# FutureSDR/FutureSDR

Hardware: NVIDIA H100
Metric: Msamples/s (higher is better)
Workload: dtype f32

## Files before the change

### futuresdr_b200/csrc/fir.cuh

```cuda
#pragma once
#include "common.cuh"

struct b2s_fir {
    b2s_ctx *ctx = nullptr;
    b2s_kind kind = B2S_C32_F32;
    size_t ntaps = 0, decim = 1;
    std::vector<float> taps_host;
    b2s_algo algo_req = B2S_ALGO_AUTO, algo = B2S_ALGO_DIRECT;

    Buf<float> d_ptaps;
    int Upad = 0;

    int tc_kblocks = 0;
    bool tc_ready = false;
    int tc_flags = 0;

    Buf<float2> d_fftH;

    Buf<double> d_taps64;
};

int32_t fir_direct_prepare(b2s_fir *f);
int32_t fir_direct_launch(b2s_fir *f, const void *d_in, size_t n_in, void *d_out, size_t n_out,
                          cudaStream_t stream);
std::vector<float> slide_table(const float *taps, size_t tf, size_t L, size_t M, size_t T, size_t lead);
bool    resamp_slide_supported(size_t L, size_t M, size_t T, size_t item_bytes);
int32_t resamp_slide_launch(b2s_ctx *ctx, b2s_kind kind, const float *d_gtab, size_t L, size_t M, size_t T,
                            const void *d_in, size_t n_in, void *d_out, size_t n_out, cudaStream_t stream);
struct FirHist {
    const void *d_hist = nullptr;
    size_t n_hist = 0;
    unsigned *publish_flag = nullptr;
    unsigned publish_value = 0;
    const unsigned *wait_flag = nullptr;
    unsigned wait_value = 0;
    unsigned *done_flag = nullptr;
    unsigned done_value = 0;
};
bool    fir_tc_supported(const b2s_fir *f);
int32_t fir_tc_launch_hist(b2s_fir *f, const FirHist *h, const void *d_in, size_t n_in, void *d_out, size_t n_out,
                           cudaStream_t stream);
int32_t fir_tc_prepare(b2s_fir *f);
int32_t fir_tc_launch(b2s_fir *f, const void *d_in, size_t n_in, void *d_out, size_t n_out,
                      cudaStream_t stream);
int32_t fir_f64_prepare(b2s_fir *f, const double *taps);
int32_t fir_f64_launch(b2s_fir *f, const void *d_in, size_t n_in, void *d_out, size_t n_out, cudaStream_t stream);
bool    fir_fft_supported(const b2s_fir *f);
int32_t fir_fft_prepare(b2s_fir *f);
int32_t fir_fft_launch(b2s_fir *f, const void *d_in, size_t n_in, void *d_out, size_t n_out,
                       cudaStream_t stream);
```

### futuresdr_b200/csrc/fir_tc.cu

```cuda
#include <cuda_bf16.h>

#include <algorithm>
#include <climits>
#include <cstdlib>
#include <type_traits>

#include "fir.cuh"

namespace {

constexpr int kStages = 2;
#ifndef B2S_RAW_SLOTS
#define B2S_RAW_SLOTS 6
#endif
constexpr int kRawSlots = B2S_RAW_SLOTS;
constexpr int kRawSlotBytes = 8192;
constexpr int kNumProducerThreads = 256;
constexpr int kNumMathThreads = 256;
constexpr int kNumLoaderThreads = 128;
constexpr int kThreadsTC = kNumMathThreads + kNumProducerThreads + kNumLoaderThreads;
constexpr int kProdWarps = kNumProducerThreads / 32;
constexpr int kMathWarps = kNumMathThreads / 32;
constexpr int kProdWarp0 = kMathWarps;
constexpr int kTmaWarp = kProdWarp0 + kProdWarps;
constexpr int kRegsAtLaunch = 65536 / kThreadsTC / 8 * 8;
constexpr int kMathRegs = 176, kProdRegs = 48, kLoaderRegs = 24;
static_assert(kNumMathThreads * kMathRegs + kNumProducerThreads * kProdRegs + kNumLoaderThreads * kLoaderRegs <=
              kThreadsTC * kRegsAtLaunch, "setmaxnreg budget exceeds the CTA's register allocation");
constexpr int kAtomsOut = 16;
constexpr int kMaxDK = 3;
constexpr int kMaxKSteps = (63 + 128 * kMaxDK - 128) / 16 + 1;
constexpr int kSplitBytesMax = (kAtomsOut + kMaxDK - 1) * 1024 * 2;
constexpr int kStageBytes = 2 * kSplitBytesMax;
constexpr int kACores = kMaxDK * 16 + 15;
constexpr int kABytes = kACores * 128;
constexpr int kSmemTC = kStages * kStageBytes + kRawSlots * kRawSlotBytes + 2 * kABytes + 1024  + 256 ;
static_assert(kSmemTC <= 227 * 1024, "tensor FIR shared memory exceeds the 227 KiB per-CTA limit");

__device__ __forceinline__ uint32_t smem_u32(const void *p) { return (uint32_t)__cvta_generic_to_shared(p); }

__device__ __forceinline__ void mbar_init(uint32_t bar, uint32_t count) {
    asm volatile("mbarrier.init.shared::cta.b64 [%0], %1;" ::"r"(bar), "r"(count));
}
__device__ __forceinline__ void mbar_arrive(uint32_t bar) {
    asm volatile("mbarrier.arrive.shared::cta.b64 _, [%0];" ::"r"(bar) : "memory");
}
__device__ __forceinline__ bool mbar_try_wait(uint32_t bar, uint32_t parity) {
    uint32_t ok;
    asm volatile(
        "{\n\t.reg .pred p;\n\t"
        "mbarrier.try_wait.parity.shared::cta.b64 p, [%1], %2;\n\t"
        "selp.b32 %0, 1, 0, p;\n\t}"
        : "=r"(ok) : "r"(bar), "r"(parity) : "memory");
    return ok != 0;
}
__device__ __forceinline__ void mbar_wait(uint32_t bar, uint32_t parity) {
    while (!mbar_try_wait(bar, parity)) {}
}
__device__ __forceinline__ bool elect_one() {
    uint32_t pred;
    asm volatile("{\n\t.reg .pred p;\n\telect.sync _|p, 0xffffffff;\n\tselp.b32 %0, 1, 0, p;\n\t}" : "=r"(pred));
    return pred != 0;
}
__device__ __forceinline__ void fence_barrier_init() { asm volatile("fence.mbarrier_init.release.cluster;" ::: "memory"); }
__device__ __forceinline__ void fence_proxy_async() { asm volatile("fence.proxy.async.shared::cta;" ::: "memory"); }

__device__ __forceinline__ void wgmma_fence() { asm volatile("wgmma.fence.sync.aligned;" ::: "memory"); }
__device__ __forceinline__ void wgmma_commit() { asm volatile("wgmma.commit_group.sync.aligned;" ::: "memory"); }
__device__ __forceinline__ void wgmma_wait_all() { asm volatile("wgmma.wait_group.sync.aligned 0;" ::: "memory"); }
__device__ __forceinline__ void st_global_if(float2 *p, float a, float b, bool pred) {
    asm volatile("{\n\t.reg .pred q;\n\tsetp.ne.b32 q, %3, 0;\n\t@q st.global.v2.f32 [%0], {%1, %2};\n\t}"
                 ::"l"(p), "f"(a), "f"(b), "r"((int)pred) : "memory");
}
__device__ __forceinline__ void st_global_if(float *p, float a, bool pred) {
    asm volatile("{\n\t.reg .pred q;\n\tsetp.ne.b32 q, %2, 0;\n\t@q st.global.f32 [%0], %1;\n\t}"
                 ::"l"(p), "f"(a), "r"((int)pred) : "memory");
}
template <int R> __device__ __forceinline__ void setmaxnreg_inc() { asm volatile("setmaxnreg.inc.sync.aligned.u32 %0;" ::"n"(R)); }
template <int R> __device__ __forceinline__ void setmaxnreg_dec() { asm volatile("setmaxnreg.dec.sync.aligned.u32 %0;" ::"n"(R)); }
__device__ __forceinline__ void wgmma_m64n128(float (&d)[64], uint64_t a_desc, uint64_t b_desc, uint32_t accumulate) {
    asm volatile(
        "{\n\t.reg .pred p;\n\t"
        "setp.ne.b32 p, %66, 0;\n\t"
        "wgmma.mma_async.sync.aligned.m64n128k16.f32.bf16.bf16 "
        "{%0, %1, %2, %3, %4, %5, %6, %7, %8, %9, %10, %11, %12, %13, %14, %15, %16, %17, %18, %19, %20, %21, %22, "
        "%23, %24, %25, %26, %27, %28, %29, %30, %31, %32, %33, %34, %35, %36, %37, %38, %39, %40, %41, %42, %43, "
        "%44, %45, %46, %47, %48, %49, %50, %51, %52, %53, %54, %55, %56, %57, %58, %59, %60, %61, %62, %63}, "
        "%64, %65, p, 1, 1, 0, 0;\n\t}"
        : "+f"(d[0]), "+f"(d[1]), "+f"(d[2]), "+f"(d[3]), "+f"(d[4]), "+f"(d[5]), "+f"(d[6]), "+f"(d[7]),
          "+f"(d[8]), "+f"(d[9]), "+f"(d[10]), "+f"(d[11]), "+f"(d[12]), "+f"(d[13]), "+f"(d[14]), "+f"(d[15]),
          "+f"(d[16]), "+f"(d[17]), "+f"(d[18]), "+f"(d[19]), "+f"(d[20]), "+f"(d[21]), "+f"(d[22]), "+f"(d[23]),
          "+f"(d[24]), "+f"(d[25]), "+f"(d[26]), "+f"(d[27]), "+f"(d[28]), "+f"(d[29]), "+f"(d[30]), "+f"(d[31]),
          "+f"(d[32]), "+f"(d[33]), "+f"(d[34]), "+f"(d[35]), "+f"(d[36]), "+f"(d[37]), "+f"(d[38]), "+f"(d[39]),
          "+f"(d[40]), "+f"(d[41]), "+f"(d[42]), "+f"(d[43]), "+f"(d[44]), "+f"(d[45]), "+f"(d[46]), "+f"(d[47]),
          "+f"(d[48]), "+f"(d[49]), "+f"(d[50]), "+f"(d[51]), "+f"(d[52]), "+f"(d[53]), "+f"(d[54]), "+f"(d[55]),
          "+f"(d[56]), "+f"(d[57]), "+f"(d[58]), "+f"(d[59]), "+f"(d[60]), "+f"(d[61]), "+f"(d[62]), "+f"(d[63])
        : "l"(a_desc), "l"(b_desc), "r"(accumulate)
        : "memory");
}
__device__ __forceinline__ void wgmma_m64n128_rs(float (&d)[64], const uint32_t (&a)[4], uint64_t b_desc,
                                                 uint32_t accumulate) {
    asm volatile(
        "{\n\t.reg .pred p;\n\t"
        "setp.ne.b32 p, %69, 0;\n\t"
        "wgmma.mma_async.sync.aligned.m64n128k16.f32.bf16.bf16 "
        "{%0, %1, %2, %3, %4, %5, %6, %7, %8, %9, %10, %11, %12, %13, %14, %15, %16, %17, %18, %19, %20, %21, %22, "
        "%23, %24, %25, %26, %27, %28, %29, %30, %31, %32, %33, %34, %35, %36, %37, %38, %39, %40, %41, %42, %43, "
        "%44, %45, %46, %47, %48, %49, %50, %51, %52, %53, %54, %55, %56, %57, %58, %59, %60, %61, %62, %63}, "
        "{%64, %65, %66, %67}, %68, p, 1, 1, 0;\n\t}"
        : "+f"(d[0]), "+f"(d[1]), "+f"(d[2]), "+f"(d[3]), "+f"(d[4]), "+f"(d[5]), "+f"(d[6]), "+f"(d[7]),
          "+f"(d[8]), "+f"(d[9]), "+f"(d[10]), "+f"(d[11]), "+f"(d[12]), "+f"(d[13]), "+f"(d[14]), "+f"(d[15]),
          "+f"(d[16]), "+f"(d[17]), "+f"(d[18]), "+f"(d[19]), "+f"(d[20]), "+f"(d[21]), "+f"(d[22]), "+f"(d[23]),
          "+f"(d[24]), "+f"(d[25]), "+f"(d[26]), "+f"(d[27]), "+f"(d[28]), "+f"(d[29]), "+f"(d[30]), "+f"(d[31]),
          "+f"(d[32]), "+f"(d[33]), "+f"(d[34]), "+f"(d[35]), "+f"(d[36]), "+f"(d[37]), "+f"(d[38]), "+f"(d[39]),
          "+f"(d[40]), "+f"(d[41]), "+f"(d[42]), "+f"(d[43]), "+f"(d[44]), "+f"(d[45]), "+f"(d[46]), "+f"(d[47]),
          "+f"(d[48]), "+f"(d[49]), "+f"(d[50]), "+f"(d[51]), "+f"(d[52]), "+f"(d[53]), "+f"(d[54]), "+f"(d[55]),
          "+f"(d[56]), "+f"(d[57]), "+f"(d[58]), "+f"(d[59]), "+f"(d[60]), "+f"(d[61]), "+f"(d[62]), "+f"(d[63])
        : "r"(a[0]), "r"(a[1]), "r"(a[2]), "r"(a[3]), "l"(b_desc), "r"(accumulate)
        : "memory");
}
__device__ __forceinline__ uint32_t ld_shared_b32(uint32_t addr) {
    uint32_t v;
    asm volatile("ld.shared.b32 %0, [%1];" : "=r"(v) : "r"(addr));
    return v;
}

__device__ __forceinline__ uint32_t cvt_bf16x2(float a, float b) {
    uint32_t r;
    asm("cvt.rn.bf16x2.f32 %0, %1, %2;" : "=r"(r) : "f"(b), "f"(a));
    return r;
}
__device__ __forceinline__ void split2(float a, float b, uint32_t &hi, uint32_t &lo) {
    hi = cvt_bf16x2(a, b);
    const float ah = __uint_as_float(hi << 16), bh = __uint_as_float(hi & 0xffff0000u);
    lo = cvt_bf16x2(a - ah, b - bh);
}

__device__ __forceinline__ uint64_t make_desc(uint32_t smem_addr, uint32_t lbo, uint32_t sbo, uint32_t layout) {
    return (uint64_t)((smem_addr & 0x3FFFF) >> 4) | ((uint64_t)(lbo >> 4) << 16) | ((uint64_t)(sbo >> 4) << 32) |
           ((uint64_t)layout << 62);
}
__device__ __forceinline__ uint64_t make_b_desc(uint32_t smem_addr) { return make_desc(smem_addr, 16, 1024, 1); }
__device__ __forceinline__ uint64_t make_a_desc(uint32_t smem_addr) { return make_desc(smem_addr, 128, 128, 0); }

struct TcParams {
    const float *in;
    float *out;
    const float *g;
    long long n_in;
    long long n_out;
    int ntaps;
    int DK;
    int num_tiles;
    int flags;
    int decim;
    const float *hist;
    int hist_items;
    int lead;
    const unsigned *wait_flag;
    unsigned wait_value;
    unsigned *done_flag;
    unsigned done_value;
    unsigned *pub_flag;
    unsigned pub_value;
    unsigned *status;
};

template <bool COMPLEX>
__global__ void __launch_bounds__(kThreadsTC, 1) fir_tc_kernel(const TcParams prm) {
    extern __shared__ unsigned char smem_raw[];
    const uint32_t raw = smem_u32(smem_raw);
    const uint32_t base = (raw + 1023u) & ~1023u;
    unsigned char *gen_base = smem_raw + (base - raw);
    const uint32_t raw_base = base + kStages * kStageBytes;
    unsigned char *raw_gen = gen_base + kStages * kStageBytes;
    const uint32_t a_base = raw_base + kRawSlots * kRawSlotBytes;
    __nv_bfloat16 *a_gen = reinterpret_cast<__nv_bfloat16 *>(raw_gen + kRawSlots * kRawSlotBytes);
    const uint32_t bar_base = a_base + 2 * kABytes;
    auto full_bar = [&](int s) { return bar_base + 8u * s; };
    auto empty_bar = [&](int s) { return bar_base + 8u * (kStages + s); };
    auto rfull_bar = [&](int r) { return bar_base + 8u * (2 * kStages + r); };
    auto rempty_bar = [&](int r) { return bar_base + 8u * (2 * kStages + kRawSlots + r); };

    const int warp = threadIdx.x >> 5, lane = threadIdx.x & 31;
    if (prm.pub_flag && blockIdx.x == 0 && threadIdx.x == 0) {
        __threadfence_system();
        asm volatile("st.release.sys.global.u32 [%0], %1;" ::"l"(prm.pub_flag), "r"(prm.pub_value) : "memory");
    }
    const int DK = prm.DK, K = 128 * DK;
    const int atoms = kAtomsOut + DK - 1;
    const int chunk_bytes = atoms * 1024;
    const int split_bytes = 2 * chunk_bytes;
    constexpr int NSEQ = COMPLEX ? 4 : 8;
    constexpr int TILE_BLOCKS = kAtomsOut * NSEQ;
    constexpr long long TILE_ITEMS = (long long)TILE_BLOCKS * 128;

    if (warp == kTmaWarp && lane == 0) {
        for (int s = 0; s < kStages; s++) { mbar_init(full_bar(s), kProdWarps); mbar_init(empty_bar(s), kMathWarps); }
        for (int r = 0; r < kRawSlots; r++) { mbar_init(rfull_bar(r), 1); mbar_init(rempty_bar(r), kProdWarps); }
        fence_barrier_init();
    }
    const int a_elems = (K / 8 + 15) * 64;
    for (int i = threadIdx.x; i < a_elems; i += kThreadsTC) {
        const int s = i >> 6, r = (i >> 3) & 7, e = i & 7;
        const int t = 8 * s + r + e - 127 - prm.lead;
        const float gv = (t >= 0 && t < prm.ntaps) ? __ldg(prm.g + t) : 0.0f;
        const __nv_bfloat16 hi = __float2bfloat16_rn(gv);
        a_gen[i] = hi;
        a_gen[kABytes / 2 + i] = __float2bfloat16_rn(gv - __bfloat162float(hi));
    }
    fence_proxy_async();
    __syncthreads();

    constexpr int F4_PER_BLOCK = COMPLEX ? 64 : 32;
    constexpr int BLOCKS_PER_SLOT = 512 / F4_PER_BLOCK;
    constexpr int SLOTS_PER_TILE = (TILE_BLOCKS + kMaxDK - 1 + BLOCKS_PER_SLOT - 1) / BLOCKS_PER_SLOT;
    constexpr int ITEM_BYTES = COMPLEX ? 8 : 4;
    const int in_blocks = TILE_BLOCKS + DK - 1;

    if (warp >= kTmaWarp) {
        setmaxnreg_dec<kLoaderRegs>();
        if (warp != kTmaWarp) return;
        if (elect_one()) {
            int rs = 0;
            uint32_t rphase = 0;
            for (int tile = blockIdx.x; tile < prm.num_tiles; tile += gridDim.x) {
                const long long item0 = (long long)tile * TILE_ITEMS;
#pragma unroll 1
                for (int s = 0; s < SLOTS_PER_TILE; s++) {
                    const int blk_first = s * BLOCKS_PER_SLOT;
                    if (blk_first >= in_blocks) break;
                    const int nblk = min(BLOCKS_PER_SLOT, in_blocks - blk_first);
                    const long long it0 = item0 + (long long)blk_first * 128;
                    long long items = (long long)nblk * 128;
                    if (it0 + items > prm.n_in) items = prm.n_in - it0;
                    long long bytes = items > 0 ? ((items * ITEM_BYTES) & ~15ll) : 0;
                    mbar_wait(rempty_bar(rs), rphase ^ 1);
                    if (tile == 0 && s == 0 && prm.hist_items > 0) {
                        if (prm.wait_flag) {
                            unsigned long long t0, t1;
                            asm volatile("mov.u64 %0, %%globaltimer;" : "=l"(t0));
                            for (;;) {
                                unsigned v;
                                asm volatile("ld.acquire.sys.global.u32 %0, [%1];" : "=r"(v) : "l"(prm.wait_flag) : "memory");
                                if ((int)(v - prm.wait_value) >= 0) break;
                                asm volatile("mov.u64 %0, %%globaltimer;" : "=l"(t1));
                                if (t1 - t0 > 4000000000ull) { atomicOr(prm.status, 1u); break; }
                                __nanosleep(64);
                            }
                            asm volatile("fence.proxy.async;" ::: "memory");
                        }
                        const uint32_t hb = (uint32_t)prm.hist_items * ITEM_BYTES;
                        const uint32_t rest = bytes > (long long)hb ? (uint32_t)bytes - hb : 0u;
                        asm volatile("mbarrier.arrive.expect_tx.shared::cta.b64 _, [%0], %1;" ::"r"(rfull_bar(rs)), "r"(hb + rest) : "memory");
                        asm volatile("cp.async.bulk.shared::cluster.global.mbarrier::complete_tx::bytes [%0], [%1], %2, [%3];"
                                     ::"r"(raw_base + rs * kRawSlotBytes), "l"(prm.hist), "r"(hb), "r"(rfull_bar(rs)) : "memory");
                        if (rest)
                            asm volatile("cp.async.bulk.shared::cluster.global.mbarrier::complete_tx::bytes [%0], [%1], %2, [%3];"
                                         ::"r"(raw_base + rs * kRawSlotBytes + hb), "l"(prm.in + (COMPLEX ? 2 : 1) * (long long)prm.hist_items),
                                           "r"(rest), "r"(rfull_bar(rs)) : "memory");
                    } else if (bytes > 0) {
                        asm volatile("mbarrier.arrive.expect_tx.shared::cta.b64 _, [%0], %1;" ::"r"(rfull_bar(rs)), "r"((uint32_t)bytes) : "memory");
                        asm volatile("cp.async.bulk.shared::cluster.global.mbarrier::complete_tx::bytes [%0], [%1], %2, [%3];"
                                     ::"r"(raw_base + rs * kRawSlotBytes), "l"(prm.in + (COMPLEX ? 2 : 1) * it0),
                                       "r"((uint32_t)bytes), "r"(rfull_bar(rs)) : "memory");
                    } else {
                        mbar_arrive(rfull_bar(rs));
                    }
                    if (++rs == kRawSlots) { rs = 0; rphase ^= 1; }
                }
            }
        }
        __syncwarp();
    } else if (warp >= kProdWarp0) {
        setmaxnreg_dec<kProdRegs>();
        const int tid = threadIdx.x - 32 * kProdWarp0;
        const int fo = tid % F4_PER_BLOCK, rowsel = tid / F4_PER_BLOCK;
        const int kc = COMPLEX ? (fo >> 5) : (fo >> 4);
        const int c16 = COMPLEX ? ((fo & 31) >> 2) : ((fo & 15) >> 1);
        const int wofs = COMPLEX ? (fo & 3) * 4 : (fo & 1) * 8;
        const uint32_t t_off = (uint32_t)(kc * chunk_bytes + wofs + rowsel * 1024);
        uint32_t xj[8];
#pragma unroll
        for (int j = 0; j < 8; j++) xj[j] = (uint32_t)(j * 128 + ((c16 ^ j) << 4));
        const bool alias_thread = rowsel < DK - 1;
        const uint32_t sb = (uint32_t)split_bytes;

        auto convert_tile = [&](auto interior_c, unsigned char *stage_ptr, long long item0, int &rs, uint32_t &rphase) {
            constexpr bool INTERIOR = decltype(interior_c)::value;
            unsigned char *tp = stage_ptr + t_off;
#pragma unroll
            for (int s = 0; s < SLOTS_PER_TILE; s++) {
                if (s * BLOCKS_PER_SLOT >= in_blocks) break;
                mbar_wait(rfull_bar(rs), rphase);
                const float4 *raw = reinterpret_cast<const float4 *>(raw_gen + rs * kRawSlotBytes);
                float4 v[2];
                v[0] = raw[tid];
                v[1] = raw[tid + 256];
                const int rs_cur = rs;
                if (++rs == kRawSlots) { rs = 0; rphase ^= 1; }
                if constexpr (!INTERIOR) {
                    if (s == 0 && item0 == 0 && tid == 0 && prm.done_flag)
                        asm volatile("st.release.sys.global.u32 [%0], %1;" ::"l"(prm.done_flag), "r"(prm.done_value) : "memory");
                }
#pragma unroll
                for (int i = 0; i < 2; i++) {
                    constexpr int ROWS = COMPLEX ? 4 : 8;
                    const int g_ct = COMPLEX ? (8 * (s & 1) + 4 * i) : (8 * i);
                    const int seq = COMPLEX ? (s >> 1) : s;
                    const bool alias_ct = COMPLEX ? ((s & 1) == 0 && i == 0 && s >= 2) : (i == 0 && s >= 1);
                    if (s == SLOTS_PER_TILE - 1) {
                        if (s * BLOCKS_PER_SLOT + rowsel + ROWS * i >= in_blocks) continue;
                    }
                    if (prm.flags & 8) continue;
                    if constexpr (!INTERIOR) {
                        const int bl = s * BLOCKS_PER_SLOT + rowsel + ROWS * i;
                        const long long it = item0 + (long long)bl * 128 + (long long)fo * (COMPLEX ? 2 : 4);
                        const long long gf = it * (COMPLEX ? 2 : 1);
                        const long long total_f = prm.n_in * (COMPLEX ? 2 : 1), copied_f = total_f & ~3ll;
                        float *e = reinterpret_cast<float *>(&v[i]);
                        const long long lead_f = (long long)prm.lead * (COMPLEX ? 2 : 1);
#pragma unroll
                        for (int c = 0; c < 4; c++) {
                            if (gf + c >= total_f || gf + c < lead_f) e[c] = 0.0f;
                            else if (gf + c >= copied_f) e[c] = prm.in[gf + c];
                        }
                    }
                    if constexpr (COMPLEX) {
                        uint32_t rh, rl, ih, il;
                        split2(v[i].x, v[i].z, rh, rl);
                        split2(v[i].y, v[i].w, ih, il);
                        if (seq < NSEQ) {
                            unsigned char *q = tp + g_ct * 1024;
                            *reinterpret_cast<uint32_t *>(q + xj[2 * (seq & 3)]) = rh;
                            *reinterpret_cast<uint32_t *>(q + xj[2 * (seq & 3)] + sb) = rl;
                            *reinterpret_cast<uint32_t *>(q + xj[2 * (seq & 3) + 1]) = ih;
                            *reinterpret_cast<uint32_t *>(q + xj[2 * (seq & 3) + 1] + sb) = il;
                        }
                        if (alias_ct && alias_thread) {
                            unsigned char *q = tp + (g_ct + kAtomsOut) * 1024;
                            *reinterpret_cast<uint32_t *>(q + xj[2 * ((seq - 1) & 3)]) = rh;
                            *reinterpret_cast<uint32_t *>(q + xj[2 * ((seq - 1) & 3)] + sb) = rl;
                            *reinterpret_cast<uint32_t *>(q + xj[2 * ((seq - 1) & 3) + 1]) = ih;
                            *reinterpret_cast<uint32_t *>(q + xj[2 * ((seq - 1) & 3) + 1] + sb) = il;
                        }
                    } else {
                        uint32_t h0, l0, h1, l1;
                        split2(v[i].x, v[i].y, h0, l0);
                        split2(v[i].z, v[i].w, h1, l1);
                        if (seq < NSEQ) {
                            unsigned char *q = tp + g_ct * 1024 + xj[seq & 7];
                            *reinterpret_cast<uint2 *>(q) = make_uint2(h0, h1);
                            *reinterpret_cast<uint2 *>(q + sb) = make_uint2(l0, l1);
                        }
                        if (alias_ct && alias_thread) {
                            unsigned char *q = tp + (g_ct + kAtomsOut) * 1024 + xj[(seq - 1) & 7];
                            *reinterpret_cast<uint2 *>(q) = make_uint2(h0, h1);
                            *reinterpret_cast<uint2 *>(q + sb) = make_uint2(l0, l1);
                        }
                    }
                }
                __syncwarp();
                if (lane == 0) mbar_arrive(rempty_bar(rs_cur));
            }
        };

        int stage = 0, rs = 0;
        uint32_t phase = 0, rphase = 0;
        for (int tile = blockIdx.x; tile < prm.num_tiles; tile += gridDim.x) {
            const long long item0 = (long long)tile * TILE_ITEMS;
            const bool interior = item0 + (long long)in_blocks * 128 <= prm.n_in &&
                                  !(tile == 0 && (prm.lead | prm.hist_items) != 0);
            mbar_wait(empty_bar(stage), phase ^ 1);
            unsigned char *stage_ptr = gen_base + stage * kStageBytes;
            if (interior) convert_tile(std::true_type{}, stage_ptr, item0, rs, rphase);
            else convert_tile(std::false_type{}, stage_ptr, item0, rs, rphase);
            fence_proxy_async();
            __syncwarp();
            if (lane == 0) mbar_arrive(full_bar(stage));
            if (++stage == kStages) { stage = 0; phase ^= 1; }
        }
    } else {
        setmaxnreg_inc<kMathRegs>();
        const int wg = __shfl_sync(0xffffffffu, warp >> 2, 0);
        const int wl = warp & 3, q4 = lane & 3;
        const int D = prm.decim, per_blk = 128 / D;
        const uint32_t a_hi = a_base + 1024u * wg, a_lo = a_hi + kABytes;
        const int p0 = 64 * (1 - wg);
        const int j0 = p0 / 16;
        const int nsteps = (prm.flags & 4) ? 0 : min((p0 + 63 + prm.lead + prm.ntaps - 1) / 16, 8 * DK - 1) - j0 + 1;

        uint32_t ghi[kMaxKSteps][4];
        {
            const uint32_t f0 = a_hi + 256u * (uint32_t)(wl + j0) + 16u * (uint32_t)(lane >> 2) + 4u * (uint32_t)q4;
#pragma unroll
            for (int i = 0; i < kMaxKSteps; i++) {
                const uint32_t f = f0 + 256u * i;
                const bool used = i < nsteps;
                ghi[i][0] = used ? ld_shared_b32(f) : 0u;
                ghi[i][1] = used ? ld_shared_b32(f + 128u) : 0u;
                ghi[i][2] = used ? ld_shared_b32(f + 128u) : 0u;
                ghi[i][3] = used ? ld_shared_b32(f + 256u) : 0u;
            }
        }

        const uint64_t a_lo_desc = make_a_desc(a_lo + 256u * j0);

        int stage = 0;
        uint32_t phase = 0;
        auto mma_tile = [&](float (&acc)[64]) {
            mbar_wait(full_bar(stage), phase);
            wgmma_fence();
            const uint64_t b_desc = make_b_desc(base + stage * kStageBytes);
#pragma unroll
            for (int i = 0; i < kMaxKSteps; i++) {
                if (i >= nsteps) break;
                const int m = (j0 >> 2) + (i >> 2);
                const uint64_t bh = b_desc + (uint32_t)(((m & 1) * chunk_bytes + (m >> 1) * 1024 + (i & 3) * 32) >> 4);
                wgmma_m64n128_rs(acc, ghi[i], bh, i != 0);
                wgmma_m64n128_rs(acc, ghi[i], bh + (uint32_t)(split_bytes >> 4), 1u);
                wgmma_m64n128(acc, a_lo_desc + 16u * i, bh, 1u);
            }
            wgmma_commit();
        };
        auto release_stage = [&]() {
            wgmma_wait_all();
            __syncwarp();
            if (lane == 0) mbar_arrive(empty_bar(stage));
            if (++stage == kStages) { stage = 0; phase ^= 1; }
        };
        const int log2D = __ffs(D) - 1;
        auto store_tile = [&](const float (&acc)[64], int tile) {
            if (prm.flags & 2) return;
#pragma unroll
            for (int h = 0; h < 2; h++) {
                const int p = 127 - (64 * wg + 16 * wl + (lane >> 2) + 8 * h);
                const int keep = (p & (D - 1)) == D - 1;
                const long long kb = ((long long)tile * TILE_BLOCKS + kAtomsOut * q4 * (COMPLEX ? 1 : 2)) * per_blk +
                                     (p >> log2D);
                const int room = (int)max(min(prm.n_out - kb, (long long)INT_MAX), 0ll) & -keep;
                const int ncols = (int)(((unsigned)room + (unsigned)per_blk - 1u) >> (7 - log2D));
                if constexpr (COMPLEX) {
#pragma unroll
                    for (int gam = 0; gam < 16; gam++)
                        st_global_if(reinterpret_cast<float2 *>(prm.out) + kb + gam * per_blk, acc[4 * gam + 2 * h],
                                     acc[4 * gam + 2 * h + 1], gam < ncols);
                } else {
#pragma unroll
                    for (int n = 0; n < 2 * kAtomsOut; n++)
                        st_global_if(prm.out + (kb + n * per_blk), acc[4 * (n % kAtomsOut) + 2 * h + n / kAtomsOut],
                                     n < ncols);
                }
            }
        };

        float acc[64];
#pragma unroll
        for (int i = 0; i < 64; i++) acc[i] = 0.0f;
        for (int tile = blockIdx.x; tile < prm.num_tiles; tile += gridDim.x) {
            mma_tile(acc);
            release_stage();
            store_tile(acc, tile);
        }
    }
}

}

bool fir_tc_supported(const b2s_fir *f) {
    if (f->decim == 0 || f->decim > 128 || 128 % f->decim != 0) return false;
    if (f->kind != B2S_C32_F32 && f->kind != B2S_F32_F32) return false;
    return f->ntaps >= 16 && f->ntaps <= 128 * kMaxDK - 127;
}

int32_t fir_tc_prepare(b2s_fir *f) {
    b2s_ctx *ctx = f->ctx;
    if (f->tc_ready) return B2S_OK;
    if (!fir_tc_supported(f)) return b2s_fail(ctx, B2S_EUNSUPPORTED, "tensor FIR: unsupported plan");
    f->tc_kblocks = (int)ceil_div(f->ntaps + 127, 128);
    B2S_CUDA(ctx, cudaFuncSetAttribute(fir_tc_kernel<true>, cudaFuncAttributeMaxDynamicSharedMemorySize, kSmemTC));
    B2S_CUDA(ctx, cudaFuncSetAttribute(fir_tc_kernel<false>, cudaFuncAttributeMaxDynamicSharedMemorySize, kSmemTC));
    for (const void *k : {(const void *)fir_tc_kernel<true>, (const void *)fir_tc_kernel<false>}) {
        cudaFuncAttributes attr;
        B2S_CUDA(ctx, cudaFuncGetAttributes(&attr, k));
        if (attr.numRegs != kRegsAtLaunch)
            return b2s_fail(ctx, B2S_EUNSUPPORTED, "tensor FIR: kernel built with %d registers per thread, its setmaxnreg "
                            "budget assumes %d", attr.numRegs, kRegsAtLaunch);
    }
    if (const char *e = getenv("B2S_TC_FLAGS")) f->tc_flags = atoi(e);
    f->tc_ready = true;
    return B2S_OK;
}

int32_t fir_tc_launch_hist(b2s_fir *f, const FirHist *h, const void *d_in, size_t n_in, void *d_out, size_t n_out,
                           cudaStream_t stream) {
    b2s_ctx *ctx = f->ctx;
    if (n_out == 0) return B2S_OK;
    if (!f->tc_ready) return b2s_fail(ctx, B2S_ESTATE, "tensor FIR not prepared");
    const bool cplx = f->kind == B2S_C32_F32;
    const size_t item = cplx ? 8 : 4, q = 16 / item;
    const uintptr_t a_in = reinterpret_cast<uintptr_t>(d_in), a_out = reinterpret_cast<uintptr_t>(d_out);
    if ((a_in % item) || (a_out % item)) return B2S_EAGAIN;
    const size_t n_hist = h ? h->n_hist : 0;
    size_t lead;
    if (n_hist) {
        const uintptr_t a_h = reinterpret_cast<uintptr_t>(h->d_hist);
        if ((a_h % item) || (a_in & 15)) return B2S_EAGAIN;
        lead = (a_h / item) % q;
        if ((lead + n_hist) % q) return B2S_EAGAIN;
        if (lead + n_hist > 1024 || n_in * item < 16) return B2S_EAGAIN;
    } else {
        lead = (a_in / item) % q;
    }
    const int DK = (int)ceil_div(f->ntaps + lead + 127, 128);
    if (DK > kMaxDK) return B2S_EAGAIN;
    TcParams prm;
    prm.lead = (int)lead;
    prm.hist_items = n_hist ? (int)(lead + n_hist) : 0;
    prm.hist = n_hist ? (const float *)h->d_hist - lead * (item / 4) : nullptr;
    prm.in = (const float *)d_in - (lead + n_hist) * (item / 4);
    prm.wait_flag = (h && n_hist) ? h->wait_flag : nullptr;
    prm.wait_value = h ? h->wait_value : 0;
    prm.done_flag = (h && n_hist) ? h->done_flag : nullptr;
    prm.done_value = h ? h->done_value : 0;
    prm.pub_flag = h ? h->publish_flag : nullptr;
    prm.pub_value = h ? h->publish_value : 0;
    prm.status = ctx->d_status;
    prm.out = (float *)d_out;
    prm.g = f->d_ptaps.get() + (size_t)f->decim * f->Upad;
    prm.n_in = (long long)(lead + n_hist + n_in);
    prm.n_out = (long long)n_out;
    prm.decim = (int)f->decim;
    prm.ntaps = (int)f->ntaps;
    prm.DK = DK;
    const long long tile_items = cplx ? 64 * 128 : 128 * 128;
    prm.num_tiles = (int)ceil_div(n_out * f->decim, (size_t)tile_items);
    prm.flags = f->tc_flags;
    const int grid = std::min(prm.num_tiles, ctx->sm_count);
    if (prm.wait_flag) ctx->flag_ops++;
    if (cplx) fir_tc_kernel<true><<<grid, kThreadsTC, kSmemTC, stream>>>(prm);
    else fir_tc_kernel<false><<<grid, kThreadsTC, kSmemTC, stream>>>(prm);
    B2S_CHECK_LAUNCH(ctx);
    return B2S_OK;
}

int32_t fir_tc_launch(b2s_fir *f, const void *d_in, size_t n_in, void *d_out, size_t n_out,
                      cudaStream_t stream) {
    const int32_t rc = fir_tc_launch_hist(f, nullptr, d_in, n_in, d_out, n_out, stream);
    if (rc == B2S_EAGAIN) return fir_direct_launch(f, d_in, n_in, d_out, n_out, stream);
    return rc;
}
```

Before: 172,000.

## Schedule tensor FIR tiles dynamically via a global atomic counter

```diff
diff --git a/futuresdr_b200/csrc/fir.cuh b/futuresdr_b200/csrc/fir.cuh
--- a/futuresdr_b200/csrc/fir.cuh
+++ b/futuresdr_b200/csrc/fir.cuh
@@ -14,6 +14,7 @@
     int tc_kblocks = 0;
     bool tc_ready = false;
     int tc_flags = 0;
+    Buf<unsigned> d_tc_sched;
 
     Buf<float2> d_fftH;
 
diff --git a/futuresdr_b200/csrc/fir_tc.cu b/futuresdr_b200/csrc/fir_tc.cu
--- a/futuresdr_b200/csrc/fir_tc.cu
+++ b/futuresdr_b200/csrc/fir_tc.cu
@@ -34,6 +34,8 @@
 constexpr int kStageBytes = 2 * kSplitBytesMax;
 constexpr int kACores = kMaxDK * 16 + 15;
 constexpr int kABytes = kACores * 128;
+constexpr int kBarBytes = 8 * (2 * kStages + 2 * kRawSlots);
+static_assert(kBarBytes + 4 * (kRawSlots + kStages) <= 256, "barriers and tile indices exceed their 256 bytes");
 constexpr int kSmemTC = kStages * kStageBytes + kRawSlots * kRawSlotBytes + 2 * kABytes + 1024  + 256 ;
 static_assert(kSmemTC <= 227 * 1024, "tensor FIR shared memory exceeds the 227 KiB per-CTA limit");
 
@@ -119,6 +121,26 @@
         : "r"(a[0]), "r"(a[1]), "r"(a[2]), "r"(a[3]), "l"(b_desc), "r"(accumulate)
         : "memory");
 }
+#ifdef B2S_TC_TIMELINE
+enum TcEvent { kTlEntry, kTlFirstCopy, kTlFirstFull, kTlFirstStore, kTlLastCopy, kTlLastStore, kTlExit, kTlEvents };
+constexpr int kTlCtas = 1024;
+__device__ unsigned long long g_tc_timeline[kTlCtas][kTlEvents];
+__device__ __forceinline__ void tl_stamp(int ev, bool pred, bool max = false) {
+    unsigned long long t;
+    asm volatile("mov.u64 %0, %%globaltimer;" : "=l"(t));
+    unsigned long long *p = &g_tc_timeline[blockIdx.x % kTlCtas][ev];
+    if (max)
+        asm volatile("{\n\t.reg .pred q;\n\tsetp.ne.b32 q, %2, 0;\n\t@q red.relaxed.gpu.global.max.u64 [%0], %1;\n\t}"
+                     ::"l"(p), "l"(t), "r"((int)pred) : "memory");
+    else
+        asm volatile("{\n\t.reg .pred q;\n\tsetp.ne.b32 q, %2, 0;\n\t@q st.global.u64 [%0], %1;\n\t}"
+                     ::"l"(p), "l"(t), "r"((int)pred) : "memory");
+}
+#define TC_STAMP(...) tl_stamp(__VA_ARGS__)
+#else
+#define TC_STAMP(...) ((void)0)
+#endif
+
 __device__ __forceinline__ uint32_t ld_shared_b32(uint32_t addr) {
     uint32_t v;
     asm volatile("ld.shared.b32 %0, [%1];" : "=r"(v) : "r"(addr));
@@ -164,6 +186,7 @@
     unsigned *pub_flag;
     unsigned pub_value;
     unsigned *status;
+    unsigned *sched;
 };
 
 template <bool COMPLEX>
@@ -181,8 +204,11 @@
     auto empty_bar = [&](int s) { return bar_base + 8u * (kStages + s); };
     auto rfull_bar = [&](int r) { return bar_base + 8u * (2 * kStages + r); };
     auto rempty_bar = [&](int r) { return bar_base + 8u * (2 * kStages + kRawSlots + r); };
+    int *slot_tile = reinterpret_cast<int *>(raw_gen + kRawSlots * kRawSlotBytes + 2 * kABytes + kBarBytes);
+    int *stage_tile = slot_tile + kRawSlots;
 
     const int warp = threadIdx.x >> 5, lane = threadIdx.x & 31;
+    TC_STAMP(kTlEntry, threadIdx.x == 0);
     if (prm.pub_flag && blockIdx.x == 0 && threadIdx.x == 0) {
         __threadfence_system();
         asm volatile("st.release.sys.global.u32 [%0], %1;" ::"l"(prm.pub_flag), "r"(prm.pub_value) : "memory");
@@ -224,7 +250,11 @@
         if (elect_one()) {
             int rs = 0;
             uint32_t rphase = 0;
-            for (int tile = blockIdx.x; tile < prm.num_tiles; tile += gridDim.x) {
+            bool first = true;
+            const int last_slot = (in_blocks + BLOCKS_PER_SLOT - 1) / BLOCKS_PER_SLOT - 1;
+            int tile = blockIdx.x;
+            while (tile < prm.num_tiles) {
+                int next = 0;
                 const long long item0 = (long long)tile * TILE_ITEMS;
 #pragma unroll 1
                 for (int s = 0; s < SLOTS_PER_TILE; s++) {
@@ -235,7 +265,9 @@
                     long long items = (long long)nblk * 128;
                     if (it0 + items > prm.n_in) items = prm.n_in - it0;
                     long long bytes = items > 0 ? ((items * ITEM_BYTES) & ~15ll) : 0;
+                    if (s == last_slot) next = (int)(gridDim.x + atomicAdd(prm.sched, 1u));
                     mbar_wait(rempty_bar(rs), rphase ^ 1);
+                    if (s == 0) slot_tile[rs] = tile;
                     if (tile == 0 && s == 0 && prm.hist_items > 0) {
                         if (prm.wait_flag) {
                             unsigned long long t0, t1;
@@ -267,11 +299,23 @@
                     } else {
                         mbar_arrive(rfull_bar(rs));
                     }
+                    TC_STAMP(kTlFirstCopy, first && s == 0);
                     if (++rs == kRawSlots) { rs = 0; rphase ^= 1; }
                 }
+                first = false;
+                tile = next;
+            }
+            TC_STAMP(kTlLastCopy, true);
+            mbar_wait(rempty_bar(rs), rphase ^ 1);
+            slot_tile[rs] = -1;
+            mbar_arrive(rfull_bar(rs));
+            if (atomicAdd(prm.sched + 1, 1u) == gridDim.x - 1) {
+                atomicExch(prm.sched, 0u);
+                atomicExch(prm.sched + 1, 0u);
             }
         }
         __syncwarp();
+        TC_STAMP(kTlExit, lane == 0, true);
     } else if (warp >= kProdWarp0) {
         setmaxnreg_dec<kProdRegs>();
         const int tid = threadIdx.x - 32 * kProdWarp0;
@@ -286,6 +330,7 @@
         const bool alias_thread = rowsel < DK - 1;
         const uint32_t sb = (uint32_t)split_bytes;
 
+        bool first = true;
         auto convert_tile = [&](auto interior_c, unsigned char *stage_ptr, long long item0, int &rs, uint32_t &rphase) {
             constexpr bool INTERIOR = decltype(interior_c)::value;
             unsigned char *tp = stage_ptr + t_off;
@@ -293,6 +338,7 @@
             for (int s = 0; s < SLOTS_PER_TILE; s++) {
                 if (s * BLOCKS_PER_SLOT >= in_blocks) break;
                 mbar_wait(rfull_bar(rs), rphase);
+                TC_STAMP(kTlFirstFull, tid == 0 && s == 0 && first);
                 const float4 *raw = reinterpret_cast<const float4 *>(raw_gen + rs * kRawSlotBytes);
                 float4 v[2];
                 v[0] = raw[tid];
@@ -367,11 +413,19 @@
 
         int stage = 0, rs = 0;
         uint32_t phase = 0, rphase = 0;
-        for (int tile = blockIdx.x; tile < prm.num_tiles; tile += gridDim.x) {
+        for (;; first = false) {
+            mbar_wait(rfull_bar(rs), rphase);
+            const int tile = slot_tile[rs];
+            mbar_wait(empty_bar(stage), phase ^ 1);
+            if (tid == 0) stage_tile[stage] = tile;
+            if (tile < 0) {
+                __syncwarp();
+                if (lane == 0) mbar_arrive(full_bar(stage));
+                break;
+            }
             const long long item0 = (long long)tile * TILE_ITEMS;
             const bool interior = item0 + (long long)in_blocks * 128 <= prm.n_in &&
                                   !(tile == 0 && (prm.lead | prm.hist_items) != 0);
-            mbar_wait(empty_bar(stage), phase ^ 1);
             unsigned char *stage_ptr = gen_base + stage * kStageBytes;
             if (interior) convert_tile(std::true_type{}, stage_ptr, item0, rs, rphase);
             else convert_tile(std::false_type{}, stage_ptr, item0, rs, rphase);
@@ -380,6 +434,7 @@
             if (lane == 0) mbar_arrive(full_bar(stage));
             if (++stage == kStages) { stage = 0; phase ^= 1; }
         }
+        TC_STAMP(kTlExit, lane == 0, true);
     } else {
         setmaxnreg_inc<kMathRegs>();
         const int wg = __shfl_sync(0xffffffffu, warp >> 2, 0);
@@ -409,7 +464,6 @@
         int stage = 0;
         uint32_t phase = 0;
         auto mma_tile = [&](float (&acc)[64]) {
-            mbar_wait(full_bar(stage), phase);
             wgmma_fence();
             const uint64_t b_desc = make_b_desc(base + stage * kStageBytes);
 #pragma unroll
@@ -457,11 +511,17 @@
         float acc[64];
 #pragma unroll
         for (int i = 0; i < 64; i++) acc[i] = 0.0f;
-        for (int tile = blockIdx.x; tile < prm.num_tiles; tile += gridDim.x) {
+        for (bool first = true;; first = false) {
+            mbar_wait(full_bar(stage), phase);
+            const int tile = __shfl_sync(0xffffffffu, stage_tile[stage], 0);
+            if (tile < 0) break;
             mma_tile(acc);
             release_stage();
+            TC_STAMP(kTlFirstStore, threadIdx.x == 0 && first);
             store_tile(acc, tile);
         }
+        TC_STAMP(kTlLastStore, lane == 0, true);
+        TC_STAMP(kTlExit, lane == 0, true);
     }
 }
 
@@ -488,6 +548,8 @@
                             "budget assumes %d", attr.numRegs, kRegsAtLaunch);
     }
     if (const char *e = getenv("B2S_TC_FLAGS")) f->tc_flags = atoi(e);
+    static const unsigned kSchedZero[2] = {0u, 0u};
+    B2S_TRY(f->d_tc_sched.upload(ctx, kSchedZero, 2, "tensor FIR tile counter"));
     f->tc_ready = true;
     return B2S_OK;
 }
@@ -526,6 +588,7 @@
     prm.pub_flag = h ? h->publish_flag : nullptr;
     prm.pub_value = h ? h->publish_value : 0;
     prm.status = ctx->d_status;
+    prm.sched = f->d_tc_sched.get();
     prm.out = (float *)d_out;
     prm.g = f->d_ptaps.get() + (size_t)f->decim * f->Upad;
     prm.n_in = (long long)(lead + n_hist + n_in);
@@ -544,6 +607,18 @@
     return B2S_OK;
 }
 
+#ifdef B2S_TC_TIMELINE
+extern "C" int fir_tc_timeline_read(unsigned long long *dst, int n_ctas) {
+    const size_t bytes = (size_t)std::min(n_ctas, kTlCtas) * kTlEvents * sizeof(unsigned long long);
+    cudaError_t e = cudaMemcpyFromSymbol(dst, g_tc_timeline, bytes);
+    if (e == cudaSuccess) {
+        static unsigned long long zeros[kTlCtas][kTlEvents];
+        e = cudaMemcpyToSymbol(g_tc_timeline, zeros, sizeof(zeros));
+    }
+    return (int)e;
+}
+#endif
+
 int32_t fir_tc_launch(b2s_fir *f, const void *d_in, size_t n_in, void *d_out, size_t n_out,
                       cudaStream_t stream) {
     const int32_t rc = fir_tc_launch_hist(f, nullptr, d_in, n_in, d_out, n_out, stream);
```

Measured after the change: 173,600, median of 6. Within noise of the previous version (+0.9%).

## Schedule tensor FIR tiles dynamically via a global atomic counter

Applied to the files above, without the earlier changes.

```diff
diff --git a/futuresdr_b200/csrc/fir.cuh b/futuresdr_b200/csrc/fir.cuh
--- a/futuresdr_b200/csrc/fir.cuh
+++ b/futuresdr_b200/csrc/fir.cuh
@@ -14,6 +14,7 @@
     int tc_kblocks = 0;
     bool tc_ready = false;
     int tc_flags = 0;
+    Buf<unsigned> d_tc_sched;
 
     Buf<float2> d_fftH;
 
diff --git a/futuresdr_b200/csrc/fir_tc.cu b/futuresdr_b200/csrc/fir_tc.cu
--- a/futuresdr_b200/csrc/fir_tc.cu
+++ b/futuresdr_b200/csrc/fir_tc.cu
@@ -64,6 +64,16 @@
 }
 __device__ __forceinline__ void fence_barrier_init() { asm volatile("fence.mbarrier_init.release.cluster;" ::: "memory"); }
 __device__ __forceinline__ void fence_proxy_async() { asm volatile("fence.proxy.async.shared::cta;" ::: "memory"); }
+#ifdef B2S_TC_TIMELINE
+__device__ unsigned long long g_tc_timeline[5][1024];
+__device__ __forceinline__ void timeline_mark(int point) {
+    unsigned long long t;
+    asm volatile("mov.u64 %0, %%globaltimer;" : "=l"(t));
+    if (blockIdx.x < 1024) g_tc_timeline[point][blockIdx.x] = t;
+}
+#else
+__device__ __forceinline__ void timeline_mark(int) {}
+#endif
 
 __device__ __forceinline__ void wgmma_fence() { asm volatile("wgmma.fence.sync.aligned;" ::: "memory"); }
 __device__ __forceinline__ void wgmma_commit() { asm volatile("wgmma.commit_group.sync.aligned;" ::: "memory"); }
@@ -152,6 +162,7 @@
     int ntaps;
     int DK;
     int num_tiles;
+    unsigned *sched;
     int flags;
     int decim;
     const float *hist;
@@ -181,8 +192,10 @@
     auto empty_bar = [&](int s) { return bar_base + 8u * (kStages + s); };
     auto rfull_bar = [&](int r) { return bar_base + 8u * (2 * kStages + r); };
     auto rempty_bar = [&](int r) { return bar_base + 8u * (2 * kStages + kRawSlots + r); };
+    volatile int *tile_ring = reinterpret_cast<volatile int *>(gen_base + (bar_base - base) + 8u * (2 * kStages + 2 * kRawSlots));
 
     const int warp = threadIdx.x >> 5, lane = threadIdx.x & 31;
+    if (threadIdx.x == 0) timeline_mark(0);
     if (prm.pub_flag && blockIdx.x == 0 && threadIdx.x == 0) {
         __threadfence_system();
         asm volatile("st.release.sys.global.u32 [%0], %1;" ::"l"(prm.pub_flag), "r"(prm.pub_value) : "memory");
@@ -224,7 +237,15 @@
         if (elect_one()) {
             int rs = 0;
             uint32_t rphase = 0;
-            for (int tile = blockIdx.x; tile < prm.num_tiles; tile += gridDim.x) {
+            for (int n = 0, tile = blockIdx.x;; n++) {
+                if (tile >= prm.num_tiles) {
+                    tile_ring[n & 3] = -1;
+                    mbar_wait(rempty_bar(rs), rphase ^ 1);
+                    mbar_arrive(rfull_bar(rs));
+                    break;
+                }
+                tile_ring[n & 3] = tile;
+                const int next = (int)gridDim.x + (int)atomicAdd(prm.sched, 1u);
                 const long long item0 = (long long)tile * TILE_ITEMS;
 #pragma unroll 1
                 for (int s = 0; s < SLOTS_PER_TILE; s++) {
@@ -236,6 +257,7 @@
                     if (it0 + items > prm.n_in) items = prm.n_in - it0;
                     long long bytes = items > 0 ? ((items * ITEM_BYTES) & ~15ll) : 0;
                     mbar_wait(rempty_bar(rs), rphase ^ 1);
+                    if (tile == (int)blockIdx.x && s == 0) timeline_mark(1);
                     if (tile == 0 && s == 0 && prm.hist_items > 0) {
                         if (prm.wait_flag) {
                             unsigned long long t0, t1;
@@ -269,6 +291,12 @@
                     }
                     if (++rs == kRawSlots) { rs = 0; rphase ^= 1; }
                 }
+                tile = next;
+            }
+            __threadfence();
+            if (atomicAdd(prm.sched + 1, 1u) == gridDim.x - 1) {
+                prm.sched[0] = 0;
+                prm.sched[1] = 0;
             }
         }
         __syncwarp();
@@ -367,11 +395,18 @@
 
         int stage = 0, rs = 0;
         uint32_t phase = 0, rphase = 0;
-        for (int tile = blockIdx.x; tile < prm.num_tiles; tile += gridDim.x) {
+        for (int n = 0;; n++) {
+            mbar_wait(rfull_bar(rs), rphase);
+            const int tile = tile_ring[n & 3];
+            mbar_wait(empty_bar(stage), phase ^ 1);
+            if (tile < 0) {
+                __syncwarp();
+                if (lane == 0) mbar_arrive(full_bar(stage));
+                break;
+            }
             const long long item0 = (long long)tile * TILE_ITEMS;
             const bool interior = item0 + (long long)in_blocks * 128 <= prm.n_in &&
                                   !(tile == 0 && (prm.lead | prm.hist_items) != 0);
-            mbar_wait(empty_bar(stage), phase ^ 1);
             unsigned char *stage_ptr = gen_base + stage * kStageBytes;
             if (interior) convert_tile(std::true_type{}, stage_ptr, item0, rs, rphase);
             else convert_tile(std::false_type{}, stage_ptr, item0, rs, rphase);
@@ -457,11 +492,16 @@
         float acc[64];
 #pragma unroll
         for (int i = 0; i < 64; i++) acc[i] = 0.0f;
-        for (int tile = blockIdx.x; tile < prm.num_tiles; tile += gridDim.x) {
+        for (int n = 0;; n++) {
+            mbar_wait(full_bar(stage), phase);
+            const int tile = __shfl_sync(0xffffffffu, tile_ring[n & 3], 0);
+            if (tile < 0) break;
             mma_tile(acc);
             release_stage();
+            if (threadIdx.x == 0) timeline_mark(tile == (int)blockIdx.x ? 2 : 3);
             store_tile(acc, tile);
         }
+        if (threadIdx.x == 0) timeline_mark(4);
     }
 }
 
@@ -488,6 +528,8 @@
                             "budget assumes %d", attr.numRegs, kRegsAtLaunch);
     }
     if (const char *e = getenv("B2S_TC_FLAGS")) f->tc_flags = atoi(e);
+    B2S_TRY(f->d_tc_sched.alloc(ctx, 2, "tensor FIR tile schedule"));
+    B2S_CUDA(ctx, cudaMemsetAsync(f->d_tc_sched.get(), 0, 2 * sizeof(unsigned), ctx->stream));
     f->tc_ready = true;
     return B2S_OK;
 }
@@ -536,6 +578,7 @@
     const long long tile_items = cplx ? 64 * 128 : 128 * 128;
     prm.num_tiles = (int)ceil_div(n_out * f->decim, (size_t)tile_items);
     prm.flags = f->tc_flags;
+    prm.sched = f->d_tc_sched.get();
     const int grid = std::min(prm.num_tiles, ctx->sm_count);
     if (prm.wait_flag) ctx->flag_ops++;
     if (cplx) fir_tc_kernel<true><<<grid, kThreadsTC, kSmemTC, stream>>>(prm);
@@ -550,3 +593,10 @@
     if (rc == B2S_EAGAIN) return fir_direct_launch(f, d_in, n_in, d_out, n_out, stream);
     return rc;
 }
+
+#ifdef B2S_TC_TIMELINE
+extern "C" __attribute__((visibility("default"))) int32_t b2s_tc_timeline_read(unsigned long long *host) {
+    if (cudaDeviceSynchronize() != cudaSuccess) return B2S_ECUDA;
+    return cudaMemcpyFromSymbol(host, g_tc_timeline, sizeof(g_tc_timeline)) == cudaSuccess ? B2S_OK : B2S_ECUDA;
+}
+#endif
```

Measured after the change: 170,200 before, 172,200 after (median of 6 runs). +1.2%, better.
